# zcablii/RS_detection

Measured on NVIDIA B200. Metric: tiles/s (Oriented R-CNN rotated-box hot path: RoIAlignRotated fwd + obb2poly + per-class nms_rotated), higher is better.
Workload: dtype f32

## Files before the change

### rs_detection_b200/csrc/roi_align.cu

```cuda
#include <cuda.h>

#include <cstdlib>
#include <mutex>

#include "common.cuh"

namespace rsdet {

constexpr int kRoiThreads = 256;
constexpr int kMaxSamples = 1024;

struct LevelSet {
    const float* feat[RSDET_MAX_LEVELS];
    float* grad[RSDET_MAX_LEVELS];
    int H[RSDET_MAX_LEVELS], W[RSDET_MAX_LEVELS];
    float scale[RSDET_MAX_LEVELS];
    int num_levels, batch, C;
    int PH, PW, sampling_ratio, version;
    float extend_w, extend_h, finest_scale;
    int dbg_drop;
    unsigned dbg_mask;
    int dbg_skip_main;
};

// ... 38 lines not shown
        }
    }
    __syncthreads();
#pragma unroll
    for (int k = 0; k < 4; k++) {
        const int idx = tid + 256 * k;
        const int cc = idx >> 4, rr = (idx & 15) * 4;
        const int gc = q0 + cc, gr = r0 + rr;
        if (gc < srcCols) {
            if (vec_out && gr + 3 < srcRows) {
                const float4 v = make_float4(tile[rr][cc], tile[rr + 1][cc], tile[rr + 2][cc], tile[rr + 3][cc]);
                *reinterpret_cast<float4*>(dst + (size_t)gc * srcRows + gr) = v;
            } else {
                for (int e = 0; e < 4; e++)
                    if (gr + e < srcRows) dst[(size_t)gc * srcRows + gr + e] = tile[rr + e][cc];
            }
        }
    }
}

template <bool TO_NHWC>
__global__ void __launch_bounds__(256) transpose_kernel(TransposeJob job) {
    __shared__ float tile[64][65];
    transpose_tile<TO_NHWC>(job, blockIdx.x, tile);
}

struct LevelSet;
struct RoiGeom;
struct PrepArgs {
    const LevelSet* L;
    const float* rois;
    int K;
    int* order;
    RoiGeom* geoms = nullptr;
    int32_t* levels_out = nullptr;
    unsigned* counter = nullptr;
};
static int launch_transpose(bool to_nhwc, const float* const* src, float* const* dst, const int* H, const int* W, int L, int N,
                            int C, cudaStream_t st, const PrepArgs* prep = nullptr);

struct alignas(16) RoiGeom {
    int batch, level, gh, gw;
    float cw, ch, bin_h, bin_w, start_h, start_w, cosv, sinv;
};

__device__ __forceinline__ int roi_level(float w, float h, const LevelSet& L) {
    if (L.num_levels <= 1) return 0;
    float s = sqrtf(__fmul_rn(w, h));
    float t = floorf(log2f(__fadd_rn(__fdiv_rn(s, L.finest_scale), 1e-6f)));
    t = fminf(fmaxf(t, 0.f), (float)(L.num_levels - 1));
    return (int)t;
}
__device__ __forceinline__ int roi_level(const float* __restrict__ r, const LevelSet& L) {
    return roi_level(__fmul_rn(L.extend_w, r[3]), __fmul_rn(L.extend_h, r[4]), L);
}
__device__ __forceinline__ RoiGeom roi_geometry(const float* __restrict__ r, const LevelSet& L) {
    RoiGeom g;
    g.batch = (int)r[0];
    float w = __fmul_rn(L.extend_w, r[3]);
    float h = __fmul_rn(L.extend_h, r[4]);
    const int lvl = roi_level(w, h, L);
    g.level = lvl;
    const float sc = L.scale[lvl];
    if (L.version == 1) {
        g.cw = __fsub_rn(__fmul_rn(r[1], sc), 0.5f);
        g.ch = __fsub_rn(__fmul_rn(r[2], sc), 0.5f);
    } else {
        g.cw = __fmul_rn(r[1], sc);
        g.ch = __fmul_rn(r[2], sc);
// ... 134 lines not shown
    for (int i = tid; i < K; i += THREADS) {
        const float* r = rois + (size_t)i * 6;
        const int bkt = bucket_of(r, roi_level(r, L));
        if (i < bkt_cap) s_bkt[i] = (unsigned short)bkt;
        atomicAdd(&s_hist[bkt], 1);
    }
    __syncthreads();
    constexpr int PER = kBuckets / THREADS;
    int a[PER], sum = 0;
#pragma unroll
    for (int k = 0; k < PER; k++) { a[k] = s_hist[PER * tid + k]; sum += a[k]; }
    int x = sum;
    const int lane = tid & 31, w = tid >> 5;
    for (int o = 1; o < 32; o <<= 1) { int y = __shfl_up_sync(0xffffffffu, x, o); if (lane >= o) x += y; }
    if (lane == 31) s_warp[w] = x;
    __syncthreads();
    if (w == 0) {
        int v = lane < THREADS / 32 ? s_warp[lane] : 0;
        for (int o = 1; o < 32; o <<= 1) { int y = __shfl_up_sync(0xffffffffu, v, o); if (lane >= o) v += y; }
        s_warp[lane] = v;
    }
    __syncthreads();
    int excl = (w ? s_warp[w - 1] : 0) + x - sum;
#pragma unroll
    for (int k = 0; k < PER; k++) { s_hist[PER * tid + k] = excl; excl += a[k]; }
    __syncthreads();
    for (int i = tid; i < K; i += THREADS) {
        const float* r = rois + (size_t)i * 6;
        const int bkt = i < bkt_cap ? (int)s_bkt[i] : bucket_of(r, roi_level(r, L));
        order[atomicAdd(&s_hist[bkt], 1)] = i;
    }
}

__device__ __forceinline__ void roi_order_1024(const LevelSet& L, const float* __restrict__ rois, int K, int* __restrict__ order) {
    __shared__ int s_hist[kBuckets];
    __shared__ int s_warp[32];
    const int tid = threadIdx.x;
    for (int i = tid; i < kBuckets; i += 1024) s_hist[i] = 0;
    __syncthreads();
    auto bucket_of = [&](int i, int& lvl) {
        const float* r = rois + (size_t)i * 6;
        lvl = roi_level(r, L);
        return roi_bucket(r, lvl, L);
    };
    int cached[4] = {0, 0, 0, 0};
#pragma unroll
    for (int c = 0; c < 4; c++) {
        const int i = tid + 1024 * c;
        if (i < K) {
            int lvl;
            cached[c] = bucket_of(i, lvl);
            atomicAdd(&s_hist[cached[c]], 1);
        }
    }
    for (int i = tid + 4096; i < K; i += 1024) {
        int lvl;
        atomicAdd(&s_hist[bucket_of(i, lvl)], 1);
    }
    __syncthreads();
    int a0 = s_hist[2 * tid], a1 = s_hist[2 * tid + 1];
    int sum = a0 + a1, x = sum;
    const int lane = tid & 31, w = tid >> 5;
    for (int o = 1; o < 32; o <<= 1) { int y = __shfl_up_sync(0xffffffffu, x, o); if (lane >= o) x += y; }
    if (lane == 31) s_warp[w] = x;
    __syncthreads();
    if (w == 0) {
        int v = s_warp[lane];
        for (int o = 1; o < 32; o <<= 1) { int y = __shfl_up_sync(0xffffffffu, v, o); if (lane >= o) v += y; }
        s_warp[lane] = v;
    }
    __syncthreads();
    int excl = (w ? s_warp[w - 1] : 0) + x - sum;
    s_hist[2 * tid] = excl;
    s_hist[2 * tid + 1] = excl + a0;
    __syncthreads();
#pragma unroll
    for (int c = 0; c < 4; c++) {
        const int i = tid + 1024 * c;
        if (i < K) order[atomicAdd(&s_hist[cached[c]], 1)] = i;
    }
    for (int i = tid + 4096; i < K; i += 1024) {
        int lvl;
        int bkt = bucket_of(i, lvl);
        order[atomicAdd(&s_hist[bkt], 1)] = i;
    }
}

__global__ void __launch_bounds__(1024) roi_order_kernel(LevelSet L, const float* __restrict__ rois, int K,
                                                         int* __restrict__ order) {
    roi_order_1024(L, rois, K, order);
}

__device__ __forceinline__ void roi_geometry_by_index(const LevelSet& L, const float* __restrict__ rois, int K, int i,
                                                      RoiGeom* __restrict__ geoms, int32_t* __restrict__ levels_out) {
    if (i >= K) return;
    const RoiGeom g = roi_geometry(rois + (size_t)i * 6, L);
    geoms[i] = g;
    if (levels_out) levels_out[i] = g.level;
}
__global__ void __launch_bounds__(1024) roi_prep_kernel(LevelSet L, const float* __restrict__ rois, int K, int* __restrict__ order,
                                                        RoiGeom* __restrict__ geoms, int32_t* __restrict__ levels_out,
                                                        unsigned* __restrict__ counter) {
    int gb = blockIdx.x;
    if (order) {
        if (gb == 0) { roi_order_1024(L, rois, K, order); return; }
        gb--;
    }
    if (gb == 0 && threadIdx.x == 0) *counter = 0u;
    roi_geometry_by_index(L, rois, K, gb * 1024 + threadIdx.x, geoms, levels_out);
}

__global__ void __launch_bounds__(256) transpose_prep_kernel(TransposeJob job, LevelSet L, const float* __restrict__ rois, int K,
                                                             int* __restrict__ order, RoiGeom* __restrict__ geoms,
                                                             int32_t* __restrict__ levels_out, unsigned* __restrict__ counter,
                                                             int geom_blocks) {
    __shared__ float tile[64][65];
    static_assert(sizeof(float) * 64 * 65 >= sizeof(int) * (kBuckets + 32), "the prep block borrows the transpose tile");
    if (blockIdx.x == 0) {
        int* s_hist = reinterpret_cast<int*>(&tile[0][0]);
        static_assert(kBuckets <= 65536, "bucket ids are cached as unsigned short");
        unsigned short* s_bkt = reinterpret_cast<unsigned short*>(s_hist + kBuckets + 32);
        const int bkt_cap = (int)((sizeof(float) * 64 * 65 - sizeof(int) * (kBuckets + 32)) / sizeof(unsigned short));
        roi_order_block<256>(L, rois, K, order, s_hist, s_hist + kBuckets, s_bkt, bkt_cap);
        return;
    }
    if ((int)blockIdx.x <= geom_blocks) {
        if (blockIdx.x == 1 && threadIdx.x == 0) *counter = 0u;
        roi_geometry_by_index(L, rois, K, ((int)blockIdx.x - 1) * 256 + threadIdx.x, geoms, levels_out);
        return;
    }
    transpose_tile<true>(job, blockIdx.x - 1 - geom_blocks, tile);
}

static int launch_transpose(bool to_nhwc, const float* const* src, float* const* dst, const int* H, const int* W, int L, int N,
                            int C, cudaStream_t st, const PrepArgs* prep) {
    TransposeJob job;
    job.num_levels = L; job.N = N; job.C = C;
    int total = 0;
    for (int l = 0; l < L; l++) {
        job.src[l] = src[l]; job.dst[l] = dst[l]; job.HW[l] = H[l] * W[l];
        job.tile_begin[l] = total;
        total += N * ceil_div(job.HW[l], 64) * ceil_div(C, 64);
    }
    job.tile_begin[L] = total;
    if (prep && to_nhwc) {
        const int geom_blocks = prep->geoms ? ceil_div(prep->K, 256) : 0;
        transpose_prep_kernel<<<total + 1 + geom_blocks, 256, 0, st>>>(job, *prep->L, prep->rois, prep->K, prep->order, prep->geoms,
                                                                        prep->levels_out, prep->counter, geom_blocks);
        count_launch();
        return cuda_status();
    }
    if (total == 0) return RSDET_OK;
    if (to_nhwc) transpose_kernel<true><<<total, 256, 0, st>>>(job);
    else transpose_kernel<false><<<total, 256, 0, st>>>(job);
    count_launch();
    return cuda_status();
}

static void launch_geometry(const LevelSet& L, const float* rois, int K, const int* order, RoiGeom* geoms, RoiGeom* gsorted,
                            int32_t* levels_out, cudaStream_t st) {
    roi_geometry_kernel<<<ceil_div(K, 128), 128, 0, st>>>(L, rois, K, order, geoms, gsorted, levels_out);
    count_launch();
}
static void launch_prep(const LevelSet& L, const float* rois, int K, RoiGeom* geoms, int* order, int32_t* levels_out, cudaStream_t st,
                        bool order_rides_with_transpose = false, RoiGeom* gsorted = nullptr) {
    if (order_rides_with_transpose) return;
    if (order) {
        roi_order_kernel<<<1, 1024, 0, st>>>(L, rois, K, order);
        count_launch();
    }
    launch_geometry(L, rois, K, order, geoms, gsorted, levels_out, st);
}

template <int kThreads = kRoiThreads, bool FIXED = false, int LPITCH = 17>
__device__ __forceinline__ void build_tap_lists(const RoiGeom& g, const LevelSet& L, int H, int W, int2* s_list, int* s_cnt,
                                                float* tmp, int unit, int base) {
    const int tid = threadIdx.x;
    const int PW_ = FIXED ? 7 : L.PW;
    const int nbins = FIXED ? 49 : L.PH * L.PW;
    const int spb = FIXED ? 4 : L.sampling_ratio * L.sampling_ratio;
    const int nsamp = nbins * spb, cap = 4 * spb, ntaps = nbins * cap;
// ... 259 lines not shown
        int e = 0;
#pragma unroll 1
        do {
            const bool p0 = e < cnt, p1 = e + 1 < cnt, p2 = e + 2 < cnt, p3 = e + 3 < cnt;
            float4 v00, v01, v10, v11, v20, v21, v30, v31;
            if (p0) { const float* q = tap_ptr(feat, (unsigned)en0.x); v00 = ldg_flavour_v4<FLAVOUR>(q); v01 = ldg_flavour_v4<FLAVOUR>(q + 128); }
            if (p1) { const float* q = tap_ptr(feat, (unsigned)en1.x); v10 = ldg_flavour_v4<FLAVOUR>(q); v11 = ldg_flavour_v4<FLAVOUR>(q + 128); }
            if (p2) { const float* q = tap_ptr(feat, (unsigned)en2.x); v20 = ldg_flavour_v4<FLAVOUR>(q); v21 = ldg_flavour_v4<FLAVOUR>(q + 128); }
            if (p3) { const float* q = tap_ptr(feat, (unsigned)en3.x); v30 = ldg_flavour_v4<FLAVOUR>(q); v31 = ldg_flavour_v4<FLAVOUR>(q + 128); }
            const float w0 = __int_as_float(en0.y), w1 = __int_as_float(en1.y), w2 = __int_as_float(en2.y), w3 = __int_as_float(en3.y);
            e += 4;
            const bool more = e < cnt;
            const int2* np = more ? lp + e : s_list + nbin * PITCH;
            if (!more) ncnt = s_cnt[nbin];
            en0 = np[0]; en1 = np[1]; en2 = np[2]; en3 = np[3];
            RSDET_ACC(p0, w0, v00, v01) RSDET_ACC(p1, w1, v10, v11) RSDET_ACC(p2, w2, v20, v21) RSDET_ACC(p3, w3, v30, v31)
        } while (e < cnt);
        stage(acc0, acc1, b);
        lp = s_list + nbin * PITCH;
        cnt = ncnt;
    }
#undef RSDET_ACC
    asm volatile("fence.proxy.async.shared::cta;" ::: "memory");
    __syncthreads();
    float* __restrict__ dst = out + ((size_t)roi * C + chunk0) * NB;
    if ((((size_t)out) & 15) == 0 && ((C * NB) & 3) == 0) {
        if (tid == 0) bulk_store_evict_first(dst, s_stage, 256u * NB * 4u);
    } else {
        for (int i = tid; i < 256 * NB; i += THREADS) __stcs(dst + i, s_stage[i]);
    }
}

constexpr size_t kStage77pOffset = (8 * 49 * 18 + 16 + 48 + 127) & ~(size_t)127;
template <int WARPS, int MINB, int TAPS = 4>
__global__ void __launch_bounds__(32 * WARPS, MINB)
roi_align_fwd77p_kernel(LevelSet L, const int* __restrict__ order, const RoiGeom* __restrict__ geoms, int K, int chunks,
                        float* __restrict__ out, unsigned* __restrict__ counter) {
    constexpr int NB = 49, PITCH = 18, THREADS = 32 * WARPS;
    extern __shared__ __align__(16) unsigned char smem_raw[];
    const int tid = threadIdx.x, lane = tid & 31, warp = tid >> 5;
    int2* s_list = reinterpret_cast<int2*>(smem_raw);
    volatile int* s_next = reinterpret_cast<volatile int*>(smem_raw + 8 * NB * PITCH);
    volatile int* s_roi = reinterpret_cast<volatile int*>(smem_raw + 8 * NB * PITCH + 4);
    const RoiGeom* s_geom = reinterpret_cast<const RoiGeom*>(smem_raw + 8 * NB * PITCH + 16);
    float* s_stage = reinterpret_cast<float*>(smem_raw + kStage77pOffset);
    const int C = L.C, items = K * chunks;
    const int oct = (lane >> 3) & 3;
    float* const sbase = s_stage + lane * 4 * NB;
    int idx = blockIdx.x;
    if (tid < 3 && idx < items) {
        const int r = order ? order[idx / chunks] : idx / chunks;
        reinterpret_cast<float4*>(smem_raw + 8 * NB * PITCH + 16)[tid] = reinterpret_cast<const float4*>(geoms + r)[tid];
        if (tid == 0) *s_roi = r;
    }
    __syncthreads();
#pragma unroll 1
    while (idx < items) {
        RoiGeom g = *s_geom;
        const int roi = *s_roi;
        g.gh = 2; g.gw = 2;
        const int chunk0 = (idx % chunks) * 256;
        const int H = L.H[g.level], W = L.W[g.level];
        if (tid < NB * 4) {
            const int b = tid >> 2, q = tid & 3;
            const int ph = b / 7, pw = b - ph * 7, iy = q >> 1, ix = q & 1;
            float x, y;
            sample_xy(g, L.version, ph, pw, iy, ix, x, y);
            const Taps t = make_taps(H, W, y, x);
#pragma unroll
            for (int k = 0; k < 4; k++) s_list[b * PITCH + q * 4 + k] = make_int2(t.o[k] * (C >> 2), __float_as_int(t.w[k]));
        }
        __syncthreads();
        if (tid < NB) {
            const int b = tid;
            int o[16];
            float w[16];
#pragma unroll
            for (int j = 0; j < 16; j++) { const int2 e = s_list[b * PITCH + j]; o[j] = e.x; w[j] = __int_as_float(e.y); }
            int pos = 0;
#pragma unroll
            for (int j = 0; j < 16; j++) {
                float acc = w[j];
#pragma unroll
                for (int i = 0; i < 16; i++) {
                    if (i <= j) continue;
                    const bool same = o[i] == o[j] && w[j] != 0.f;
                    acc += same ? w[i] : 0.f;
                    w[i] = same ? 0.f : w[i];
                }
                if (w[j] != 0.f) s_list[b * PITCH + pos++] = make_int2(o[j], __float_as_int(acc));
            }
#ifdef RSDET_TUNING
            if (L.dbg_drop > 1) {
                int q = 0;
                for (int e = 0; e < pos; e++)
                    if ((e + b) % L.dbg_drop != 0) s_list[b * PITCH + q++] = s_list[b * PITCH + e];
                pos = q;
            }
#endif
            s_list[b * PITCH + 16] = make_int2(pos, 0);
        }
        if (tid == THREADS - 1) {
            asm volatile("cp.async.bulk.wait_group.read 0;" ::: "memory");
            *s_next = (int)(atomicAdd(counter, 1u) + gridDim.x);
        }
        __syncthreads();
        if (tid < 3 && *s_next < items) {
            const int nidx = *s_next;
            const int r = order ? __ldg(order + nidx / chunks) : nidx / chunks;
            if (tid == 0) *s_roi = r;
            asm volatile("cp.async.ca.shared.global [%0], [%1], 16;" ::"r"((unsigned)__cvta_generic_to_shared(s_geom) + 16u * tid),
                         "l"(reinterpret_cast<const char*>(geoms + r) + 16 * tid) : "memory");
            asm volatile("cp.async.commit_group;" ::: "memory");
        }

        const float4* __restrict__ feat =
            reinterpret_cast<const float4*>(L.feat[g.level] + (size_t)g.batch * H * W * C + chunk0) + lane;
        auto stage = [&](float4 a0, float4 a1, int b) {
            a0.x *= 0.25f; a0.y *= 0.25f; a0.z *= 0.25f; a0.w *= 0.25f;
            a1.x *= 0.25f; a1.y *= 0.25f; a1.z *= 0.25f; a1.w *= 0.25f;
            const float4 r0 = rot4(a0, oct), r1 = rot4(a1, oct);
            float* const sb = sbase + b;
            float* const q0 = sb + ((0 + oct) & 3) * NB;
            float* const q1 = sb + ((1 + oct) & 3) * NB;
            float* const q2 = sb + ((2 + oct) & 3) * NB;
            float* const q3 = sb + ((3 + oct) & 3) * NB;
            q0[0] = r0.x; q1[0] = r0.y; q2[0] = r0.z; q3[0] = r0.w;
            q0[128 * NB] = r1.x; q1[128 * NB] = r1.y; q2[128 * NB] = r1.z; q3[128 * NB] = r1.w;
        };
        const int2* lp = s_list + warp * PITCH;
        int4 en[TAPS / 2];
#pragma unroll
        for (int t = 0; t < TAPS / 2; t++) en[t] = reinterpret_cast<const int4*>(lp)[t];
        int cnt = lp[16].x;
#pragma unroll 1
        for (int b = warp; b < NB; b += WARPS) {
            float4 acc0 = make_float4(0.f, 0.f, 0.f, 0.f), acc1 = acc0;
            const int nbin = min(b + WARPS, NB - 1);
            int ncnt = cnt;
            int e = 0;
#pragma unroll 1
            do {
                float4 va[TAPS], vb[TAPS];
                float wt[TAPS];
#pragma unroll
                for (int t = 0; t < TAPS; t++) {
                    const int off = (t & 1) ? en[t >> 1].z : en[t >> 1].x;
                    wt[t] = __int_as_float((t & 1) ? en[t >> 1].w : en[t >> 1].y);
                    if (e + t < cnt) { const float* q = tap_ptr(feat, (unsigned)off); va[t] = ldg_nc_v4(q); vb[t] = ldg_nc_v4(q + 128); }
                }
                const int e0 = e;
                e += TAPS;
                const bool more = e < cnt;
                const int2* np = more ? lp + e : s_list + nbin * PITCH;
                if (!more) ncnt = s_list[nbin * PITCH + 16].x;
#pragma unroll
                for (int t = 0; t < TAPS / 2; t++) en[t] = reinterpret_cast<const int4*>(np)[t];
#pragma unroll
                for (int t = 0; t < TAPS; t++)
                    if (e0 + t < cnt) {
                        acc0.x = fmaf(wt[t], va[t].x, acc0.x); acc0.y = fmaf(wt[t], va[t].y, acc0.y); acc0.z = fmaf(wt[t], va[t].z, acc0.z); acc0.w = fmaf(wt[t], va[t].w, acc0.w);
                        acc1.x = fmaf(wt[t], vb[t].x, acc1.x); acc1.y = fmaf(wt[t], vb[t].y, acc1.y); acc1.z = fmaf(wt[t], vb[t].z, acc1.z); acc1.w = fmaf(wt[t], vb[t].w, acc1.w);
                    }
            } while (e < cnt);
            stage(acc0, acc1, b);
            lp = s_list + nbin * PITCH;
            cnt = ncnt;
        }
        if (tid < 3) asm volatile("cp.async.wait_all;" ::: "memory");
        asm volatile("fence.proxy.async.shared::cta;" ::: "memory");
        __syncthreads();
        if (tid == THREADS - 1) {
            unsigned long long pol;
            asm volatile("createpolicy.fractional.L2::evict_first.b64 %0, 1.0;" : "=l"(pol));
            asm volatile("cp.async.bulk.global.shared::cta.bulk_group.L2::cache_hint [%0], [%1], %2, %3;"
                         ::"l"(out + ((size_t)roi * C + chunk0) * NB), "r"((unsigned)__cvta_generic_to_shared(s_stage)), "r"(256u * NB * 4u), "l"(pol) : "memory");
            asm volatile("cp.async.bulk.commit_group;" ::: "memory");
        }
        idx = *s_next;
    }
    if (tid == THREADS - 1) asm volatile("cp.async.bulk.wait_group.read 0;" ::: "memory");
}

static void set_dyn_smem(const void* func, size_t bytes) {
    struct Slot { const void* f; size_t b; };
    static Slot slots[64][16];
    static std::mutex mu;
    int dev = 0;
    cudaGetDevice(&dev);
    std::lock_guard<std::mutex> lk(mu);
    if (dev < 0 || dev >= 64) { cudaFuncSetAttribute(func, cudaFuncAttributeMaxDynamicSharedMemorySize, (int)bytes); return; }
    for (int i = 0; i < 16; i++) {
        Slot& s = slots[dev][i];
        if (s.f == func || s.f == nullptr) {
            if (s.f == func && s.b >= bytes) return;
            s.f = func; s.b = bytes;
            cudaFuncSetAttribute(func, cudaFuncAttributeMaxDynamicSharedMemorySize, (int)bytes);
            return;
        }
    }
    cudaFuncSetAttribute(func, cudaFuncAttributeMaxDynamicSharedMemorySize, (int)bytes);
}

static int roi_path_choice() {
#ifdef RSDET_TUNING
    if (const char* e = getenv("RSDET_ROI_PATH")) return atoi(e);
#endif
    return 1;
}

static bool fast_path_ok(const rsdet_roi_align_cfg* c);
static size_t fwd_smem_bytes(const rsdet_roi_align_cfg* c);
static thread_local cudaEvent_t t_prof_start = nullptr, t_prof_stop = nullptr;
struct GatherTimer {
    cudaStream_t st;
    cudaEvent_t stop;
    explicit GatherTimer(cudaStream_t s) : st(s), stop(t_prof_stop) {
        if (t_prof_start && t_prof_stop) cudaEventRecord(t_prof_start, st); else stop = nullptr;
        t_prof_start = t_prof_stop = nullptr;
    }
    ~GatherTimer() { if (stop) cudaEventRecord(stop, st); }
};

static bool fwd77_ok(const rsdet_roi_align_cfg* c) {
    return c->pooled_h == 7 && c->pooled_w == 7 && c->sampling_ratio == 2 && c->channels % 256 == 0;
}
#ifdef RSDET_TUNING
#include "roi_align_tuning.cuh"
#endif

template <int QPT>
__global__ void __launch_bounds__(kRoiThreads, 4)
roi_align_bwd_kernel(LevelSet L, const float* __restrict__ rois, const int* __restrict__ order, const RoiGeom* __restrict__ geoms,
                     int K, const float* __restrict__ grad_out) {
    extern __shared__ __align__(16) unsigned char smem_raw[];
    const int roi = order ? order[blockIdx.x] : blockIdx.x;
    const int tid = threadIdx.x;
    const int nbins = L.PH * L.PW;
    const int spb = L.sampling_ratio * L.sampling_ratio;
    const int cap = 4 * spb;
    const int C = L.C;
    const int Q = quads_per_chunk(C);
    const int chunk0 = blockIdx.y * Q * 4;
    const int Qc = min(Q, (C - chunk0) / 4);
    int2* s_list = reinterpret_cast<int2*>(smem_raw);
    int* s_cnt = reinterpret_cast<int*>(smem_raw + list_bytes(nbins, cap));
    float* s_stage = reinterpret_cast<float*>(smem_raw + list_bytes(nbins, cap) + ((nbins * 4 + 15) & ~15));
    __shared__ RoiGeom s_g;

    if (!geoms) {
        if (tid == 0) s_g = roi_geometry(rois + (size_t)roi * 6, L);
        __syncthreads();
    }
    const RoiGeom g = geoms ? geoms[roi] : s_g;
    const int H = L.H[g.level], W = L.W[g.level];
// ... 135 lines not shown
        L.feat[l] = nullptr; L.grad[l] = nullptr;
        L.H[l] = l < c->num_levels ? c->height[l] : 1;
        L.W[l] = l < c->num_levels ? c->width[l] : 1;
        L.scale[l] = l < c->num_levels ? c->spatial_scale[l] : 1.f;
    }
    return L;
}

static size_t fwd_smem_bytes(const rsdet_roi_align_cfg* c) {
    size_t nbins = (size_t)c->pooled_h * c->pooled_w;
    size_t ntaps = nbins * 4 * c->sampling_ratio * c->sampling_ratio;
    size_t stage = sizeof(float) * 4 * nbins * quads_per_chunk(c->channels), tmp = 12 * (ntaps + nbins);
    return list_bytes(nbins, ntaps / nbins) + ((nbins * 4 + 15) & ~(size_t)15) + (stage > tmp ? stage : tmp);
}

}

using namespace rsdet;

extern "C" size_t rsdet_roi_align_rotated_workspace_bytes(const rsdet_roi_align_cfg* cfg, int num_rois, int backward) {
    (void)backward;
    if (check_cfg(cfg) != RSDET_OK) return 0;
    size_t b = ws_bytes<int>(num_rois > 0 ? num_rois : 1) + ws_bytes<RoiGeom>(num_rois > 0 ? num_rois : 1) +
               ws_bytes<RoiGeom>((num_rois > 0 ? num_rois : 1) + 1);
#ifdef RSDET_TUNING
    if (fast_path_ok(cfg) && split_path_ok(cfg))
        b += ws_bytes<unsigned char>((size_t)(num_rois > 0 ? num_rois : 1) *
                                     (rec_stride((size_t)cfg->pooled_h * cfg->pooled_w, 4 * (size_t)cfg->sampling_ratio * cfg->sampling_ratio) +
                                      stream_rec_stride((size_t)cfg->pooled_h * cfg->pooled_w, 4 * (size_t)cfg->sampling_ratio * cfg->sampling_ratio)));
#endif
    if (cfg->channels_last || !fast_path_ok(cfg)) return b + 256;
    for (int l = 0; l < cfg->num_levels; l++)
        b += ws_bytes<float>((size_t)cfg->batch * cfg->channels * cfg->height[l] * cfg->width[l]);
    return b + 256;
}

extern "C" int rsdet_roi_align_rotated_forward(const rsdet_roi_align_cfg* cfg, const float* const* feats_host, const float* rois,
                                               int num_rois, float* out, int32_t* levels_out, void* workspace,
                                               size_t workspace_bytes, void* stream) {
    int rc = check_cfg(cfg);
    if (rc != RSDET_OK) return rc;
    if (num_rois < 0) return RSDET_EINVAL;
    if (num_rois == 0) return RSDET_OK;
    if (!feats_host || !rois || !out) return RSDET_EINVAL;
    for (int l = 0; l < cfg->num_levels; l++)
        if (!feats_host[l]) return RSDET_EINVAL;
    cudaStream_t st = (cudaStream_t)stream;
    LevelSet L = make_levels(cfg);
    if (!fast_path_ok(cfg)) {
        GenericMaps M;
        M.channels_last = cfg->channels_last;
        for (int l = 0; l < RSDET_MAX_LEVELS; l++) { M.feat[l] = l < cfg->num_levels ? feats_host[l] : nullptr; M.grad[l] = nullptr; }
        long long total = (long long)num_rois * cfg->channels * cfg->pooled_h * cfg->pooled_w;
        int grid = (int)(ceil_div_ll(total, 256) < (long long)kNumSMs * 16 ? ceil_div_ll(total, 256) : (long long)kNumSMs * 16);
        roi_align_generic_kernel<false><<<grid, 256, 0, st>>>(L, M, rois, num_rois, out, levels_out);
        count_launch();
        return cuda_status();
    }
    if (workspace_bytes < rsdet_roi_align_rotated_workspace_bytes(cfg, num_rois, 0)) return RSDET_EWORKSPACE;
    Workspace ws(workspace, workspace_bytes);
    int* order_ws = ws.take<int>(num_rois);
    RoiGeom* geoms = ws.take<RoiGeom>(num_rois);
    RoiGeom* gsorted = ws.take<RoiGeom>(num_rois + 1);
    if (cfg->channels_last) {
        for (int l = 0; l < cfg->num_levels; l++) L.feat[l] = feats_host[l];
    } else {
        float* dst[RSDET_MAX_LEVELS];
        for (int l = 0; l < cfg->num_levels; l++) {
            dst[l] = ws.take<float>((size_t)cfg->batch * cfg->channels * cfg->height[l] * cfg->width[l]);
            L.feat[l] = dst[l];
        }
        if (!ws.ok()) return RSDET_EWORKSPACE;
    }
    int* order = num_rois >= 256 && order_ws ? order_ws : nullptr;
#ifdef RSDET_TUNING
    if (getenv("RSDET_ROI_NOORDER")) order = nullptr;
#endif
    const bool ride = !cfg->channels_last && order && num_rois <= kPrepMaxRois;
    bool lean = fwd77_ok(cfg) && roi_path_choice() == 1 && (((size_t)out) & 15) == 0;
#ifdef RSDET_TUNING
    if (getenv("RSDET_ROI_NOPERSIST") || getenv("RSDET_ROI_V8") || getenv("RSDET_ROI_MINB3") || getenv("RSDET_ROI_Q") ||
        getenv("RSDET_ROI_LD") || getenv("RSDET_ROI_WARPS") || getenv("RSDET_ROI_OLDPREP"))
        lean = false;
#endif
    unsigned* const counter = reinterpret_cast<unsigned*>(gsorted + num_rois);
    if (!lean) launch_prep(L, rois, num_rois, geoms, order, levels_out, st, ride, gsorted);
    else if (!ride) {
        roi_prep_kernel<<<(order ? 1 : 0) + ceil_div(num_rois, 1024), 1024, 0, st>>>(L, rois, num_rois, order, geoms, levels_out, counter);
        count_launch();
    }
    if (!cfg->channels_last) {
        PrepArgs prep = {&L, rois, num_rois, order};
        if (lean) { prep.geoms = geoms; prep.levels_out = levels_out; prep.counter = counter; }
        float* dst[RSDET_MAX_LEVELS];
        for (int l = 0; l < cfg->num_levels; l++) dst[l] = const_cast<float*>(L.feat[l]);
        rc = launch_transpose(true, feats_host, dst, cfg->height, cfg->width, cfg->num_levels, cfg->batch, cfg->channels, st,
                              ride ? &prep : nullptr);
        if (rc != RSDET_OK) return rc;
        if (ride && !lean) launch_geometry(L, rois, num_rois, order, geoms, gsorted, levels_out, st);
    }
    size_t smem = fwd_smem_bytes(cfg);
#ifdef RSDET_TUNING
    if (const char* e = getenv("RSDET_ROI_PAD_SMEM")) smem += (size_t)atoi(e) * 1024;
#endif
    set_dyn_smem((const void*)roi_align_fwd_kernel<1>, smem);
    set_dyn_smem((const void*)roi_align_fwd_kernel<2>, smem);
#ifdef RSDET_TUNING
    {
        int trc = RSDET_OK;
        if (tuning_forward(cfg, L, ws, rois, order, geoms, num_rois, out, levels_out, st, &trc)) return trc;
    }
#endif
    GatherTimer gather_timer(st);
    if (fwd77_ok(cfg) && roi_path_choice() == 1) {
        smem = smem - fwd_smem_bytes(cfg) + kStage77Offset + sizeof(float) * 49 * 256;
        int warps = 7;
#ifdef RSDET_TUNING
        if (const char* e = getenv("RSDET_ROI_WARPS")) warps = atoi(e);
#endif
#ifdef RSDET_TUNING
        const int flavour = getenv("RSDET_ROI_LD") ? atoi(getenv("RSDET_ROI_LD")) : 0;
        dim3 g77(num_rois, cfg->channels / 256);
        if (flavour == 1) { set_dyn_smem((const void*)roi_align_fwd77_kernel<8, 1>, smem); roi_align_fwd77_kernel<8, 1><<<g77, 256, smem, st>>>(L, gsorted, num_rois, out); count_launch(); return cuda_status(); }
        if (flavour == 2) { set_dyn_smem((const void*)roi_align_fwd77_kernel<8, 2>, smem); roi_align_fwd77_kernel<8, 2><<<g77, 256, smem, st>>>(L, gsorted, num_rois, out); count_launch(); return cuda_status(); }
        if (flavour == 3) { set_dyn_smem((const void*)roi_align_fwd77_kernel<8, 3>, smem); roi_align_fwd77_kernel<8, 3><<<g77, 256, smem, st>>>(L, gsorted, num_rois, out); count_launch(); return cuda_status(); }
#endif
// ... 46 lines not shown
            }
            count_launch();
            return cuda_status();
        }
#endif
        if (lean) {
            const int chunks = cfg->channels / 256;
            const long long items = (long long)num_rois * chunks;
            int ctas = kNumSMs * 3;
#ifdef RSDET_TUNING
            if (const char* e = getenv("RSDET_ROI_PCTAS")) ctas = atoi(e);
#endif
#ifdef RSDET_TUNING
            if (const char* e = getenv("RSDET_ROI_PVAR")) {
                const size_t smv = kStage77pOffset + sizeof(float) * 49 * 256;
                unsigned* ctr = reinterpret_cast<unsigned*>(gsorted + num_rois);
                const int v = atoi(e);
#define RSDET_PV(W_, M_, T_) { const int grid = (int)(items < kNumSMs * M_ ? items : kNumSMs * M_); \
                               set_dyn_smem((const void*)roi_align_fwd77p_kernel<W_, M_, T_>, smv); \
                               roi_align_fwd77p_kernel<W_, M_, T_><<<grid, 32 * W_, smv, st>>>(L, order, geoms, num_rois, chunks, out, ctr); \
                               count_launch(); return cuda_status(); }
                if (v == 1062) RSDET_PV(10, 2, 6)
                if (v == 1262) RSDET_PV(12, 2, 6)
                if (v == 882) RSDET_PV(8, 2, 8)
                if (v == 1082) RSDET_PV(10, 2, 8)
                if (v == 763) RSDET_PV(7, 3, 6)
                if (v == 863) RSDET_PV(8, 3, 6)
                if (v == 1442) RSDET_PV(14, 2, 4)
                if (v == 1242) RSDET_PV(12, 2, 4)
#undef RSDET_PV
            }
#endif
            const size_t smp = kStage77pOffset + sizeof(float) * 49 * 256;
            set_dyn_smem((const void*)roi_align_fwd77p_kernel<8, 3>, smp);
            roi_align_fwd77p_kernel<8, 3><<<(int)(items < ctas ? items : ctas), 256, smp, st>>>(
                L, order, geoms, num_rois, chunks, out, counter);
            count_launch();
            return cuda_status();
        }
        if (warps == 7) {
            set_dyn_smem((const void*)roi_align_fwd77_kernel<7>, smem);
            roi_align_fwd77_kernel<7><<<dim3(num_rois, cfg->channels / 256), 224, smem, st>>>(L, gsorted, num_rois, out);
        } else {
            set_dyn_smem((const void*)roi_align_fwd77_kernel<8>, smem);
            roi_align_fwd77_kernel<8><<<dim3(num_rois, cfg->channels / 256), 256, smem, st>>>(L, gsorted, num_rois, out);
        }
        count_launch();
        return cuda_status();
    }
    const int Q = quads_per_chunk(cfg->channels);
    dim3 grid(num_rois, ceil_div(cfg->channels / 4, Q));
    if (cfg->channels % 256 == 0)
        roi_align_fwd_kernel<2><<<grid, kRoiThreads, smem, st>>>(L, rois, order, geoms, num_rois, out, nullptr);
    else
        roi_align_fwd_kernel<1><<<grid, kRoiThreads, smem, st>>>(L, rois, order, geoms, num_rois, out, nullptr);
    count_launch();
    return cuda_status();
}

extern "C" int rsdet_roi_align_rotated_backward(const rsdet_roi_align_cfg* cfg, const float* grad_out, const float* rois,
                                                int num_rois, float* const* grad_feats_host, void* workspace,
                                                size_t workspace_bytes, void* stream) {
    int rc = check_cfg(cfg);
    if (rc != RSDET_OK) return rc;
    if (num_rois < 0 || !grad_feats_host) return RSDET_EINVAL;
    for (int l = 0; l < cfg->num_levels; l++)
// ... 77 lines not shown
```

Baseline: 5677.

## Fuse NCHW-to-NHWC feature transpose into persistent RoIAlign kernel with per-image readiness flags

Removes the separate transpose(+prep) launch on the lean NCHW path. The persistent 7x7 RoIAlign kernel now pulls copy tasks (48-pixel by 256-channel transposes) and RoI work items from one atomic work queue, interleaved per image. Each image's RoI work waits on a release/acquire counter for that image's copies. This overlaps the layout conversion with gathers and saves a launch, at the cost of spin-waits, coherent (non-.nc) feature loads, a host-mapped timeout flag, and possible deadlock risk if copy tasks are starved.

```diff
diff --git a/rs_detection_b200/csrc/roi_align.cu b/rs_detection_b200/csrc/roi_align.cu
--- a/rs_detection_b200/csrc/roi_align.cu
+++ b/rs_detection_b200/csrc/roi_align.cu
@@ -94,9 +94,6 @@
     const float* rois;
     int K;
     int* order;
-    RoiGeom* geoms = nullptr;
-    int32_t* levels_out = nullptr;
-    unsigned* counter = nullptr;
 };
 static int launch_transpose(bool to_nhwc, const float* const* src, float* const* dst, const int* H, const int* W, int L, int N,
                             int C, cudaStream_t st, const PrepArgs* prep = nullptr);
@@ -297,7 +294,8 @@
     }
 }
 
-__device__ __forceinline__ void roi_order_1024(const LevelSet& L, const float* __restrict__ rois, int K, int* __restrict__ order) {
+__device__ __forceinline__ void roi_order_1024(const LevelSet& L, const float* __restrict__ rois, int K, int* __restrict__ order,
+                                               int* __restrict__ image_begin = nullptr) {
     __shared__ int s_hist[kBuckets];
     __shared__ int s_warp[32];
     const int tid = threadIdx.x;
@@ -339,6 +337,10 @@
     s_hist[2 * tid] = excl;
     s_hist[2 * tid + 1] = excl + a0;
     __syncthreads();
+    if (image_begin) {
+        if (tid <= L.batch) image_begin[tid] = tid == L.batch ? K : (L.batch > 1 ? s_hist[tid * L.num_levels * 64] : 0);
+        __syncthreads();
+    }
 #pragma unroll
     for (int c = 0; c < 4; c++) {
         const int i = tid + 1024 * c;
@@ -365,20 +367,21 @@
 }
 __global__ void __launch_bounds__(1024) roi_prep_kernel(LevelSet L, const float* __restrict__ rois, int K, int* __restrict__ order,
                                                         RoiGeom* __restrict__ geoms, int32_t* __restrict__ levels_out,
-                                                        unsigned* __restrict__ counter) {
+                                                        unsigned* __restrict__ counter, unsigned* __restrict__ copy_done = nullptr,
+                                                        int* __restrict__ image_begin = nullptr) {
     int gb = blockIdx.x;
     if (order) {
-        if (gb == 0) { roi_order_1024(L, rois, K, order); return; }
+        if (gb == 0) { roi_order_1024(L, rois, K, order, image_begin); return; }
         gb--;
     }
     if (gb == 0 && threadIdx.x == 0) *counter = 0u;
+    if (gb == 0 && copy_done)
+        for (int b = threadIdx.x; b < L.batch; b += 1024) copy_done[b] = 0u;
     roi_geometry_by_index(L, rois, K, gb * 1024 + threadIdx.x, geoms, levels_out);
 }
 
 __global__ void __launch_bounds__(256) transpose_prep_kernel(TransposeJob job, LevelSet L, const float* __restrict__ rois, int K,
-                                                             int* __restrict__ order, RoiGeom* __restrict__ geoms,
-                                                             int32_t* __restrict__ levels_out, unsigned* __restrict__ counter,
-                                                             int geom_blocks) {
+                                                             int* __restrict__ order) {
     __shared__ float tile[64][65];
     static_assert(sizeof(float) * 64 * 65 >= sizeof(int) * (kBuckets + 32), "the prep block borrows the transpose tile");
     if (blockIdx.x == 0) {
@@ -389,12 +392,7 @@
         roi_order_block<256>(L, rois, K, order, s_hist, s_hist + kBuckets, s_bkt, bkt_cap);
         return;
     }
-    if ((int)blockIdx.x <= geom_blocks) {
-        if (blockIdx.x == 1 && threadIdx.x == 0) *counter = 0u;
-        roi_geometry_by_index(L, rois, K, ((int)blockIdx.x - 1) * 256 + threadIdx.x, geoms, levels_out);
-        return;
-    }
-    transpose_tile<true>(job, blockIdx.x - 1 - geom_blocks, tile);
+    transpose_tile<true>(job, blockIdx.x - 1, tile);
 }
 
 static int launch_transpose(bool to_nhwc, const float* const* src, float* const* dst, const int* H, const int* W, int L, int N,
@@ -409,9 +407,7 @@
     }
     job.tile_begin[L] = total;
     if (prep && to_nhwc) {
-        const int geom_blocks = prep->geoms ? ceil_div(prep->K, 256) : 0;
-        transpose_prep_kernel<<<total + 1 + geom_blocks, 256, 0, st>>>(job, *prep->L, prep->rois, prep->K, prep->order, prep->geoms,
-                                                                        prep->levels_out, prep->counter, geom_blocks);
+        transpose_prep_kernel<<<total + 1, 256, 0, st>>>(job, *prep->L, prep->rois, prep->K, prep->order);
         count_launch();
         return cuda_status();
     }
@@ -737,34 +733,184 @@
 }
 
 constexpr size_t kStage77pOffset = (8 * 49 * 18 + 16 + 48 + 127) & ~(size_t)127;
-template <int WARPS, int MINB, int TAPS = 4>
+
+constexpr int kCopyPixels = 48;
+constexpr int kCopyWaitSpins = 1 << 22;
+struct CopyPlan {
+    const float* src[RSDET_MAX_LEVELS];
+    int task_begin[RSDET_MAX_LEVELS + 1];
+    int tasks;
+    int interleave;
+    const int* image_begin;
+    unsigned* done;
+    unsigned* expired;
+};
+struct SeqItem { int copy, image, index; };
+
+__device__ __forceinline__ SeqItem seq_item(long long s, const CopyPlan& P, int batch, int chunks) {
+    const long long T = P.tasks;
+    if (!P.interleave) {
+        if (s < T * batch) return {1, (int)(s / T), (int)(s % T)};
+        return {0, 0, (int)(s - T * batch)};
+    }
+    if (s < T) return {1, 0, (int)s};
+    s -= T;
+    for (int b = 0; b < batch; b++) {
+        const int p0 = __ldg(P.image_begin + b);
+        const long long G = (long long)(__ldg(P.image_begin + b + 1) - p0) * chunks;
+        const long long Tn = b + 1 < batch ? T : 0;
+        if (s < G + Tn) {
+            const long long nt = s * Tn / (G + Tn);
+            if ((s + 1) * Tn / (G + Tn) > nt) return {1, b + 1, (int)nt};
+            return {0, b, (int)((long long)p0 * chunks + s - nt)};
+        }
+        s -= G + Tn;
+    }
+    return {0, 0, 0x7fffffff};
+}
+
+__device__ __noinline__ void copy_rows(const float* __restrict__ src, float* __restrict__ dst, int HW, int C, int np, bool vec,
+                                       unsigned* done, float* tile) {
+    const int tid = threadIdx.x;
+    if (vec) {
+#pragma unroll
+        for (int h = 0; h < 2; h++) {
+            float4 v[6];
+#pragma unroll
+            for (int k = 0; k < 6; k++) {
+                const int i = tid + 256 * (6 * h + k), c = i / 12, p = (i % 12) * 4;
+                if (p < np) asm volatile("ld.global.nc.L1::no_allocate.v4.f32 {%0,%1,%2,%3}, [%4];"
+                                         : "=f"(v[k].x), "=f"(v[k].y), "=f"(v[k].z), "=f"(v[k].w) : "l"(src + (size_t)c * HW + p));
+            }
+#pragma unroll
+            for (int k = 0; k < 6; k++) {
+                const int i = tid + 256 * (6 * h + k), c = i / 12, p = (i % 12) * 4;
+                float* s = tile + c * 49 + p;
+                s[0] = v[k].x; s[1] = v[k].y; s[2] = v[k].z; s[3] = v[k].w;
+            }
+        }
+    } else {
+        for (int i = tid; i < 256 * kCopyPixels; i += 256) {
+            const int c = i / kCopyPixels, p = i % kCopyPixels;
+            if (p < np) tile[c * 49 + p] = __ldg(src + (size_t)c * HW + p);
+        }
+    }
+    __syncthreads();
+    const int cq = tid & 63, oct = (cq >> 3) & 3;
+#pragma unroll
+    for (int k = 0; k < 12; k++) {
+        const int p = (tid >> 6) + 4 * k;
+        if (p < np) {
+            const float* s = tile + 4 * cq * 49 + p;
+            float4 r;
+            r.x = s[((0 + oct) & 3) * 49]; r.y = s[((1 + oct) & 3) * 49];
+            r.z = s[((2 + oct) & 3) * 49]; r.w = s[((3 + oct) & 3) * 49];
+            *reinterpret_cast<float4*>(dst + (size_t)p * C + 4 * cq) = unrot4(r, oct);
+        }
+    }
+    __syncthreads();
+    if (tid == 0) asm volatile("red.release.gpu.global.add.u32 [%0], 1;" ::"l"(done) : "memory");
+}
+__device__ __forceinline__ void copy_task(const CopyPlan& P, const LevelSet& L, int image, int t, float* tile) {
+    int l = 0;
+    while (l + 1 < L.num_levels && t >= P.task_begin[l + 1]) l++;
+    t -= P.task_begin[l];
+    const int C = L.C, chunks = C >> 8, HW = L.H[l] * L.W[l];
+    const int p0 = (t / chunks) * kCopyPixels, c0 = (t % chunks) * 256;
+    copy_rows(P.src[l] + ((size_t)image * C + c0) * HW + p0,
+              const_cast<float*>(L.feat[l]) + ((size_t)image * HW + p0) * C + c0,
+              HW, C, min(kCopyPixels, HW - p0), (HW & 3) == 0 && ((size_t)P.src[l] & 15) == 0,
+              P.done + image, tile);
+}
+
+__device__ __forceinline__ void wait_copy_done(const CopyPlan& P, int image, unsigned tasks, volatile unsigned* s_ready) {
+    if (image < 32 && ((*s_ready >> image) & 1u)) return;
+    unsigned v;
+    for (int spins = 0;; spins++) {
+        asm volatile("ld.relaxed.gpu.global.u32 %0, [%1];" : "=r"(v) : "l"(P.done + image) : "memory");
+        if (v >= tasks) break;
+        if (spins == kCopyWaitSpins) {
+            if (P.expired) *reinterpret_cast<volatile unsigned*>(P.expired) = 1u;
+            return;
+        }
+        __nanosleep(256);
+    }
+    asm volatile("ld.acquire.gpu.global.u32 %0, [%1];" : "=r"(v) : "l"(P.done + image) : "memory");
+    if (image < 32) *s_ready = *s_ready | (1u << image);
+}
+
+template <bool NC>
+__device__ __forceinline__ float4 ld_feat_v4(const float* p) {
+    if (NC) return ldg_nc_v4(p);
+    float4 r;
+    asm volatile("ld.global.v4.f32 {%0,%1,%2,%3}, [%4];" : "=f"(r.x), "=f"(r.y), "=f"(r.z), "=f"(r.w) : "l"(p));
+    return r;
+}
+
+template <int WARPS, int MINB, int TAPS = 4, bool COPY = false>
 __global__ void __launch_bounds__(32 * WARPS, MINB)
 roi_align_fwd77p_kernel(LevelSet L, const int* __restrict__ order, const RoiGeom* __restrict__ geoms, int K, int chunks,
-                        float* __restrict__ out, unsigned* __restrict__ counter) {
+                        float* __restrict__ out, unsigned* __restrict__ counter, CopyPlan P = CopyPlan()) {
     constexpr int NB = 49, PITCH = 18, THREADS = 32 * WARPS;
+    static_assert(!COPY || THREADS == 256, "copy tasks are written for 256 threads");
     extern __shared__ __align__(16) unsigned char smem_raw[];
     const int tid = threadIdx.x, lane = tid & 31, warp = tid >> 5;
     int2* s_list = reinterpret_cast<int2*>(smem_raw);
     volatile int* s_next = reinterpret_cast<volatile int*>(smem_raw + 8 * NB * PITCH);
     volatile int* s_roi = reinterpret_cast<volatile int*>(smem_raw + 8 * NB * PITCH + 4);
+    volatile int* s_item = reinterpret_cast<volatile int*>(smem_raw + 8 * NB * PITCH + 64);
+    volatile unsigned* s_ready = reinterpret_cast<volatile unsigned*>(smem_raw + 8 * NB * PITCH + 76);
     const RoiGeom* s_geom = reinterpret_cast<const RoiGeom*>(smem_raw + 8 * NB * PITCH + 16);
     float* s_stage = reinterpret_cast<float*>(smem_raw + kStage77pOffset);
-    const int C = L.C, items = K * chunks;
+    const int C = L.C, items = COPY ? P.tasks * L.batch + K * chunks : K * chunks;
     const int oct = (lane >> 3) & 3;
     float* const sbase = s_stage + lane * 4 * NB;
-    int idx = blockIdx.x;
-    if (tid < 3 && idx < items) {
-        const int r = order ? order[idx / chunks] : idx / chunks;
+    const unsigned first = COPY ? 0u : gridDim.x;
+    if (COPY && tid == 0) *s_next = (int)atomicAdd(counter, 1u);
+    if (COPY) __syncthreads();
+    int idx = COPY ? *s_next : (int)blockIdx.x;
+    SeqItem it = {0, 0, idx};
+    if (COPY) it = seq_item(idx, P, L.batch, chunks);
+    if (COPY && tid == THREADS - 2) *s_ready = 0u;
+    if (tid < 3 && idx < items && !it.copy) {
+        const int r = order ? order[it.index / chunks] : it.index / chunks;
         reinterpret_cast<float4*>(smem_raw + 8 * NB * PITCH + 16)[tid] = reinterpret_cast<const float4*>(geoms + r)[tid];
         if (tid == 0) *s_roi = r;
     }
     __syncthreads();
 #pragma unroll 1
     while (idx < items) {
+        if (COPY && it.copy) {
+            int n = 0;
+            SeqItem nx = {0, 0, 0};
+            if (tid == THREADS - 1) {
+                asm volatile("cp.async.bulk.wait_group.read 0;" ::: "memory");
+                n = (int)(atomicAdd(counter, 1u) + first);
+                nx = seq_item(n, P, L.batch, chunks);
+            }
+            __syncthreads();
+            if (tid == THREADS - 1) { *s_next = n; s_item[0] = nx.copy; s_item[1] = nx.image; s_item[2] = nx.index; }
+            __syncthreads();
+            const int nidx = *s_next;
+            const SeqItem ni = {s_item[0], s_item[1], s_item[2]};
+            if (tid < 3 && nidx < items && !ni.copy) {
+                const int r = order ? __ldg(order + ni.index / chunks) : ni.index / chunks;
+                if (tid == 0) *s_roi = r;
+                asm volatile("cp.async.ca.shared.global [%0], [%1], 16;" ::"r"((unsigned)__cvta_generic_to_shared(s_geom) + 16u * tid),
+                             "l"(reinterpret_cast<const char*>(geoms + r) + 16 * tid) : "memory");
+                asm volatile("cp.async.commit_group;" ::: "memory");
+            }
+            copy_task(P, L, it.image, it.index, s_stage);
+            if (tid < 3) asm volatile("cp.async.wait_all;" ::: "memory");
+            __syncthreads();
+            idx = nidx;
+            it = ni;
+            continue;
+        }
         RoiGeom g = *s_geom;
         const int roi = *s_roi;
         g.gh = 2; g.gw = 2;
-        const int chunk0 = (idx % chunks) * 256;
+        const int chunk0 = (it.index % chunks) * 256;
         const int H = L.H[g.level], W = L.W[g.level];
         if (tid < NB * 4) {
             const int b = tid >> 2, q = tid & 3;
@@ -807,12 +953,19 @@
         }
         if (tid == THREADS - 1) {
             asm volatile("cp.async.bulk.wait_group.read 0;" ::: "memory");
-            *s_next = (int)(atomicAdd(counter, 1u) + gridDim.x);
-        }
+            const int n = (int)(atomicAdd(counter, 1u) + first);
+            *s_next = n;
+            if (COPY) {
+                const SeqItem ni = seq_item(n, P, L.batch, chunks);
+                s_item[0] = ni.copy; s_item[1] = ni.image; s_item[2] = ni.index;
+            }
+        }
+        if (COPY && tid == THREADS - 2)
+            wait_copy_done(P, min(max(g.batch, 0), L.batch - 1), (unsigned)P.tasks, s_ready);
         __syncthreads();
-        if (tid < 3 && *s_next < items) {
-            const int nidx = *s_next;
-            const int r = order ? __ldg(order + nidx / chunks) : nidx / chunks;
+        if (tid < 3 && *s_next < items && !(COPY && s_item[0])) {
+            const int nx = COPY ? s_item[2] : *s_next;
+            const int r = order ? __ldg(order + nx / chunks) : nx / chunks;
             if (tid == 0) *s_roi = r;
             asm volatile("cp.async.ca.shared.global [%0], [%1], 16;" ::"r"((unsigned)__cvta_generic_to_shared(s_geom) + 16u * tid),
                          "l"(reinterpret_cast<const char*>(geoms + r) + 16 * tid) : "memory");
@@ -852,7 +1005,7 @@
                 for (int t = 0; t < TAPS; t++) {
                     const int off = (t & 1) ? en[t >> 1].z : en[t >> 1].x;
                     wt[t] = __int_as_float((t & 1) ? en[t >> 1].w : en[t >> 1].y);
-                    if (e + t < cnt) { const float* q = tap_ptr(feat, (unsigned)off); va[t] = ldg_nc_v4(q); vb[t] = ldg_nc_v4(q + 128); }
+                    if (e + t < cnt) { const float* q = tap_ptr(feat, (unsigned)off); va[t] = ld_feat_v4<!COPY>(q); vb[t] = ld_feat_v4<!COPY>(q + 128); }
                 }
                 const int e0 = e;
                 e += TAPS;
@@ -883,6 +1036,8 @@
             asm volatile("cp.async.bulk.commit_group;" ::: "memory");
         }
         idx = *s_next;
+        if (COPY) it = {s_item[0], s_item[1], s_item[2]};
+        else it.index = idx;
     }
     if (tid == THREADS - 1) asm volatile("cp.async.bulk.wait_group.read 0;" ::: "memory");
 }
@@ -926,6 +1081,29 @@
     }
     ~GatherTimer() { if (stop) cudaEventRecord(stop, st); }
 };
+
+static unsigned* g_copy_wait_flag = nullptr;
+static std::mutex g_copy_wait_mu;
+static unsigned* copy_wait_flag(cudaStream_t st) {
+    std::lock_guard<std::mutex> lk(g_copy_wait_mu);
+    if (!g_copy_wait_flag) {
+        cudaStreamCaptureStatus cs = cudaStreamCaptureStatusNone;
+        if (cudaStreamIsCapturing(st, &cs) != cudaSuccess || cs != cudaStreamCaptureStatusNone) { cudaGetLastError(); return nullptr; }
+        void* p = nullptr;
+        if (cudaHostAlloc(&p, sizeof(unsigned), cudaHostAllocMapped | cudaHostAllocPortable) != cudaSuccess) { cudaGetLastError(); return nullptr; }
+        *static_cast<volatile unsigned*>(p) = 0u;
+        g_copy_wait_flag = static_cast<unsigned*>(p);
+    }
+    return g_copy_wait_flag;
+}
+static int copy_wait_status() {
+    std::lock_guard<std::mutex> lk(g_copy_wait_mu);
+    if (g_copy_wait_flag && *static_cast<volatile unsigned*>(g_copy_wait_flag)) {
+        *static_cast<volatile unsigned*>(g_copy_wait_flag) = 0u;
+        return (int)cudaErrorLaunchTimeout;
+    }
+    return RSDET_OK;
+}
 
 static bool fwd77_ok(const rsdet_roi_align_cfg* c) {
     return c->pooled_h == 7 && c->pooled_w == 7 && c->sampling_ratio == 2 && c->channels % 256 == 0;
@@ -1127,6 +1305,7 @@
     if (cfg->channels_last || !fast_path_ok(cfg)) return b + 256;
     for (int l = 0; l < cfg->num_levels; l++)
         b += ws_bytes<float>((size_t)cfg->batch * cfg->channels * cfg->height[l] * cfg->width[l]);
+    b += ws_bytes<unsigned>(cfg->batch) + ws_bytes<int>((size_t)cfg->batch + 1);
     return b + 256;
 }
 
@@ -1157,6 +1336,8 @@
     int* order_ws = ws.take<int>(num_rois);
     RoiGeom* geoms = ws.take<RoiGeom>(num_rois);
     RoiGeom* gsorted = ws.take<RoiGeom>(num_rois + 1);
+    unsigned* copy_done = nullptr;
+    int* image_begin = nullptr;
     if (cfg->channels_last) {
         for (int l = 0; l < cfg->num_levels; l++) L.feat[l] = feats_host[l];
     } else {
@@ -1165,6 +1346,8 @@
             dst[l] = ws.take<float>((size_t)cfg->batch * cfg->channels * cfg->height[l] * cfg->width[l]);
             L.feat[l] = dst[l];
         }
+        copy_done = ws.take<unsigned>(cfg->batch);
+        image_begin = ws.take<int>((size_t)cfg->batch + 1);
         if (!ws.ok()) return RSDET_EWORKSPACE;
     }
     int* order = num_rois >= 256 && order_ws ? order_ws : nullptr;
@@ -1179,14 +1362,21 @@
         lean = false;
 #endif
     unsigned* const counter = reinterpret_cast<unsigned*>(gsorted + num_rois);
-    if (!lean) launch_prep(L, rois, num_rois, geoms, order, levels_out, st, ride, gsorted);
+    const bool copy_in_kernel = lean && !cfg->channels_last;
+    const bool batch_major = order && (cfg->batch == 1 || (cfg->num_levels * 64 <= kBuckets && cfg->batch <= kBuckets / (cfg->num_levels * 64)));
+    if (copy_in_kernel) {
+        rc = copy_wait_status();
+        if (rc != RSDET_OK) return rc;
+        roi_prep_kernel<<<(order ? 1 : 0) + ceil_div(num_rois, 1024), 1024, 0, st>>>(L, rois, num_rois, order, geoms, levels_out, counter,
+                                                                                      copy_done, batch_major ? image_begin : nullptr);
+        count_launch();
+    } else if (!lean) launch_prep(L, rois, num_rois, geoms, order, levels_out, st, ride, gsorted);
     else if (!ride) {
         roi_prep_kernel<<<(order ? 1 : 0) + ceil_div(num_rois, 1024), 1024, 0, st>>>(L, rois, num_rois, order, geoms, levels_out, counter);
         count_launch();
     }
-    if (!cfg->channels_last) {
+    if (!cfg->channels_last && !copy_in_kernel) {
         PrepArgs prep = {&L, rois, num_rois, order};
-        if (lean) { prep.geoms = geoms; prep.levels_out = levels_out; prep.counter = counter; }
         float* dst[RSDET_MAX_LEVELS];
         for (int l = 0; l < cfg->num_levels; l++) dst[l] = const_cast<float*>(L.feat[l]);
         rc = launch_transpose(true, feats_host, dst, cfg->height, cfg->width, cfg->num_levels, cfg->batch, cfg->channels, st,
@@ -1299,6 +1489,30 @@
             }
 #endif
             const size_t smp = kStage77pOffset + sizeof(float) * 49 * 256;
+            if (copy_in_kernel) {
+                CopyPlan P;
+                int tasks = 0;
+                for (int l = 0; l < RSDET_MAX_LEVELS; l++) {
+                    P.src[l] = l < cfg->num_levels ? feats_host[l] : nullptr;
+                    P.task_begin[l] = tasks;
+                    if (l < cfg->num_levels) tasks += ceil_div(cfg->height[l] * cfg->width[l], kCopyPixels) * chunks;
+                }
+                P.task_begin[RSDET_MAX_LEVELS] = tasks;
+                P.tasks = tasks;
+                P.interleave = batch_major ? 1 : 0;
+#ifdef RSDET_TUNING
+                if (getenv("RSDET_ROI_COPY_FIRST")) P.interleave = 0;
+#endif
+                P.image_begin = image_begin;
+                P.done = copy_done;
+                P.expired = copy_wait_flag(st);
+                const long long all = items + (long long)tasks * cfg->batch;
+                set_dyn_smem((const void*)roi_align_fwd77p_kernel<8, 3, 4, true>, smp);
+                roi_align_fwd77p_kernel<8, 3, 4, true><<<(int)(all < ctas ? all : ctas), 256, smp, st>>>(
+                    L, order, geoms, num_rois, chunks, out, counter, P);
+                count_launch();
+                return cuda_status();
+            }
             set_dyn_smem((const void*)roi_align_fwd77p_kernel<8, 3>, smp);
             roi_align_fwd77p_kernel<8, 3><<<(int)(items < ctas ? items : ctas), 256, smp, st>>>(
                 L, order, geoms, num_rois, chunks, out, counter);
```

New measurement: 4583, median of 6. -19.3%, worse.
